# Dingyf717/target-allocation-ppo-transformer

Measured on AMD Instinct MI355X. Metric: env-steps/sec (whole node), full PPO rollout, 4096 envs x 16 UAV x 32 tgt per GPU, higher is better.
Workload: dtype f32 policy (f32 MFMA + fp32-accurate split products on the f16 MFMA) + f64 env

## Files before the change

target-allocation-ppo-transformer_amd/csrc/policy_block.hpp:

```cpp
#pragma once
#include "policy_encoder.hpp"

namespace uavhip {
namespace pol {

template <int head, int nout, int DQ = 4, int XT = (S - 1) * SPW>
__device__ void head_mlp(TID_F Smem& sm, const float* __restrict__ P, const APre<DQ>& pw, float* out) {
    const float* W0 = P + kOffs.o[head + 0];
    const float* b0 = P + kOffs.o[head + 1];
    const float* W2 = P + kOffs.o[head + 2];
    const float* b2 = P + kOffs.o[head + 3];
    const int wv = TIDX() >> 6;
    constexpr int kItems = SPW * nout;
    const int item = TIDX() >> 4, k4 = TIDX() & 15;
    const int p = item / nout, a = (item - p * nout) % nout;
    const f32x4 w2 = *reinterpret_cast<const f32x4*>(W2 + a * HID + 4 * k4);
    const float bb2 = b2[a];
    if (wv < HID / 16) linear1<1, true, DQ>(TID_C pw, W0, D, b0, 16 * wv, sm.h, LDH, XT, sm.z, LDZ, 16 * wv, 0);
    __syncthreads();
    if (item < kItems) {
        const f32x4 z = *reinterpret_cast<const f32x4*>(sm.z + p * LDZ + 4 * k4);
        float acc = (w2.x * z.x + w2.y * z.y) + (w2.z * z.z + w2.w * z.w);
        acc = add_xor2(add_xor1(acc));
        acc += __int_as_float(__builtin_amdgcn_mov_dpp(__float_as_int(acc), 0x141, 0xF, 0xF, true));
// ... 194 lines not shown
    static_assert(!AONLY || (ROWS && ENV && !TR && !VONLY), "actor only: the inference ring forward + env step");
    int blk = bx, role = VONLY ? 2 : AONLY ? 1 : 0;
    if constexpr (TR) {
        if (io.split) {
            role = blk < io.split ? 1 : 2;
            if (role == 2) blk -= io.split;
        }
    }
    const bool do_actor = role != 2, do_critic = role != 1;
    const int b0 = blk * SPW;
    [[maybe_unused]] bool critic_first = false;
    if constexpr (TR) critic_first = role == 0 && io.mix && ((blk >> 3) & 1);
    PTR(0);
    [[maybe_unused]] EmbPre ep_a, ep_c;
    [[maybe_unused]] KvPre<kActorTrunk, 0, TR> pkv_a;
    [[maybe_unused]] KvPre<kCriticTrunk, 0, TR> pkv_c;
    if constexpr (TR) {
        if (do_actor && !critic_first) {
            ep_a = embed_load<kActorTrunk>(TID_C P);
            pkv_a = kv_prefetch<kActorTrunk, 0, TR>(TID_C P);
        } else {
            ep_c = embed_load<kCriticTrunk>(TID_C P);
            pkv_c = kv_prefetch<kCriticTrunk, 0, TR>(TID_C P);
        }
    }
    gather_windows<TR, ROWS>(TID_C sm, states, B, io, b0, do_actor, P + kRangeOff);
    if constexpr (!TR) {
        const int pd = (int)TIDX() - (NTHR - kWave);
        if (!actions_in && pd >= 0 && pd < SPW) {
            const unsigned long long c = offset + (offset_dev ? *offset_dev : 0ull) + (unsigned long long)(b0 + pd);
            const u32x4 r = philox(u32x4{(uint32_t)c, (uint32_t)(c >> 32), 0x5eedu, 0x9e37u}, (uint32_t)seed,
                                   (uint32_t)(seed >> 32));
            sm.u01[pd] = u01f(r.x);
            if constexpr (AONLY) {
                if (greedy_stride > 0 && (b0 + pd) % greedy_stride == 0) sm.u01[pd] = -1.f;
            }
        }
    }
    __syncthreads();
    PTR(1);
    if (!ROWS || !do_actor) {
        const float xm = a0f_from_tmax(TID_C sm);
        if (TR && TIDX() == 0 && io.xmax) io.xmax[blk] = xm;
    }
    if (TR && blk == 0 && TIDX() < kRtN && io.rtab_out) io.rtab_out[TIDX()] = sm.rtab[TIDX()];
    const int wv = TIDX() >> 6;
    const float* headw_a = P + kOffs.o[kActorHead];
    const float* headw_c = P + kOffs.o[kCriticHead];
    [[maybe_unused]] const bool env_grp =
        (ENV & kEnvGrp) && env.N <= envgrp::L && env.M <= envgrp::L && b0 + 2 * wv + 1 < B;
    [[maybe_unused]] envgrp::GRegs gR;
    [[maybe_unused]] envgrp::GPending gq;
    if constexpr (ROWS) {
        if (do_actor) {
            RingPre<kActorTrunk> pw[3];
            RowPre<2> rp;
            rows_prologue<kActorTrunk>(TID_C sm, P, pw, rp, rio, b0, [&] { a0f_from_tmax(TID_C sm); });
            PTR(2);
            __syncthreads();
            encoder_layer_rows<kActorTrunk>(TID_C sm, P, pw, rp, rio, b0);
        }
    }
    constexpr int kHd = TR ? 2 : 4;
    APre<kHd> ph;
    [[maybe_unused]] auto actor = [&] {
        if constexpr (TR && !ROWS) {
            embed_apply<kActorTrunk, TR, kEmbH, split_kv<kActorTrunk, 0, TR>()>(TID_C sm, ep_a, io.e[0],
                                                                                           nullptr, b0);
            PTR(2);
            __syncthreads();
            auto hook = [&] {
                if (wv < 4) ph = prefetch<kHd>(TID_C headw_a, D, 16 * wv, 0);
                if (do_critic && !critic_first) {
                    ep_c = embed_load<kCriticTrunk>(TID_C P);
                    pkv_c = kv_prefetch<kCriticTrunk, 0, TR>(TID_C P);
                }
            };
            encoder_layer<kActorTrunk, 0, true, TR, decltype(hook)>(TID_C sm, P, pkv_a, io.L[0], b0, hook);
            __syncthreads();
            PTR(3);
            head_mlp<kActorHead, 2, kHd>(TID_C sm, P, ph, sm.logits);
            store_hidden(TID_C sm, io.z[0], b0);
        }
    };
    if constexpr (TR) {
        if (do_actor && !critic_first) actor();
    } else if (do_actor) {
        if constexpr (!ROWS) {
            APre<2> pkv = prefetch<2>(TID_C P + kOffs.o[layer_param(kActorTrunk, 0, INW)], D, kv_row(wv, 0), 0);
            embed<kActorTrunk, TR>(TID_C sm, P, io.e[0], nullptr, b0);
            PTR(2);
            __syncthreads();
            encoder_layer<kActorTrunk, 0, true, TR>(TID_C sm, P, pkv, io.L[0], b0);
        }
        if constexpr (AONLY && (ENV & kEnvGrp) && !kExpNoEnv) {
            if (env_grp) {
                const int le = tid_env() & 63;
                envgrp::gload_issue(gR, gq, env, b0 + 2 * (int)(tid_env() >> 6) + (le >> 5), le & 31);
            }
        }
        if (wv < 4) ph = prefetch<kHd>(TID_C headw_a, D, 16 * wv, 0);
        __syncthreads();
        PTR(3);
        head_mlp<kActorHead, 2, kHd>(TID_C sm, P, ph, sm.logits);
    }
    PTR(4);
    if (do_critic) {
// ... 166 lines not shown
```

target-allocation-ppo-transformer_amd/csrc/policy_encoder.hpp:

```cpp
#pragma once
#include "policy_core.hpp"

namespace uavhip {
namespace pol {

struct LnOut {
    float *x, *h, *rs;
    int b0, compact;
    bool nt = true;
};
__device__ __forceinline__ int trow(int tok, int b0) { return (b0 + (tok & (SPW - 1))) * S + tok / SPW; }
__device__ __forceinline__ int orow(int tok, int b0, bool compact) {
    return compact ? b0 + (tok & (SPW - 1)) : trow(tok, b0);
}

struct LnPar {
    f32x4 bb, ww, lb;
};
__device__ __forceinline__ f32x4 ln_bias(TID_F const float* __restrict__ bias) {
    return *reinterpret_cast<const f32x4*>(bias + 16 * (TIDX() >> 6) + 4 * (LANE() >> 4));
}
__device__ __forceinline__ LnPar ln_load(TID_F const f32x4 bb, const float* __restrict__ w, const float* __restrict__ b) {
    const int f0 = 16 * (TIDX() >> 6) + 4 * (LANE() >> 4);
    return LnPar{bb, *reinterpret_cast<const f32x4*>(w + f0), *reinterpret_cast<const f32x4*>(b + f0)};
// ... 130 lines not shown
        }
    }
}
__device__ __forceinline__ void attention_full_store(TID_F Smem& sm, int c, const f32x4 (&o)[3], float sc) {
    const int q4 = TIDX() & 3, task = TIDX() >> 2;
    const int hh = task & 3, p = (task >> 2) & 15, grp = task >> 6;
    const int d0 = hh * HD + 4 * q4, qs0 = grp ? 3 : 0, nq = grp ? 2 : 3;
#pragma unroll
    for (int qi = 0; qi < 3; ++qi) {
        if (qi < nq) {
            const int ti = (qs0 + qi) * SPW + p;
            hsplit_store(reinterpret_cast<_Float16*>(sm.ctx), psw(ti, 4 * c * HD + d0), o[qi] * sc);
        }
    }
}
template <int trunk, int layer>
__device__ void attention_full(TID_F Smem& sm, int c, const float* __restrict__ P = nullptr) {
    f32x4 o[3];
    attention_full_core(TID_C sm, c, o);
    attention_full_store(TID_C sm, c, o, att_sc<trunk, layer>(sm, (int)((TIDX() >> 4) & 15)).sc);
}

__device__ __forceinline__ void attention_task(TID_F Smem& sm, int task, int qs0, f32x4& o, int& ti, int& d0) {
    const int q4 = TIDX() & 3;
    const int hh = task & 3, rest = task >> 2, p = rest & 15, si = qs0 + (rest >> 4);
    ti = si * SPW + p;
    d0 = hh * HD + 4 * q4;
    const f32x4 q = *reinterpret_cast<const f32x4*>(sm.big + ti * LDB + d0) * kAttQ;
    float sc[S];
    float mx = -INFINITY;
#pragma unroll
    for (int j = 0; j < S; ++j) {
        const f32x4 k = *reinterpret_cast<const f32x4*>(sm.big + (j * SPW + p) * LDB + 64 + d0);
        float part = att_dot(q, k);
        part = add_xor2(add_xor1(part));
        sc[j] = sm.mask[p * S + j] ? -INFINITY : part;
        mx = j ? fmaxf(mx, sc[j]) : sc[j];
    }
    float den = 0.f;
#pragma unroll
    for (int j = 0; j < S; ++j) {
        sc[j] = __expf(sc[j] - mx);
        den = j ? den + sc[j] : sc[j];
    }
    const float inv = att_recip(den);
    f32x4 v[S];
#pragma unroll
    for (int j = 0; j < S; ++j) v[j] = *reinterpret_cast<const f32x4*>(sm.big + (j * SPW + p) * LDB + 128 + d0);
    o = f32x4{0.f, 0.f, 0.f, 0.f};
    att_mix(o, sc, inv, v);
}
__device__ __forceinline__ void attention_out(TID_F Smem& sm, int c, int ti, int d0, const f32x4 o, float sc) {
    hsplit_store(reinterpret_cast<_Float16*>(sm.ctx), psw(ti, 4 * c * HD + d0), o * sc);
}
template <int trunk, int layer>
__device__ void attention_chunk(TID_F Smem& sm, int c, int qs0, int nqs, const float* __restrict__ P = nullptr) {
    const int ntask = nqs * SPW * 4;
    for (int task = TIDX() >> 2; task < ntask; task += NTHR / 4) {
        f32x4 o;
        int ti, d0;
        attention_task(TID_C sm, task, qs0, o, ti, d0);
        attention_out(TID_C sm, c, ti, d0, o, att_sc<trunk, layer>(sm, ti & 15).sc);
    }
}

struct EmbPre {
    f32x4 a, bb, pp[S];
};
template <int trunk>
__device__ __forceinline__ EmbPre embed_load(TID_F const float* __restrict__ P) {
    const float* We = P + kOffs.o[trunk + EMB_W];
    const float* be = P + kOffs.o[trunk + EMB_B];
    const float* pos = P + kOffs.o[trunk + POS];
    const int l = LANE(), i16 = l & 15, g = l >> 4, wv = TIDX() >> 6;
    const int f = 16 * wv + i16;
    EmbPre r;
    r.a.x = 4 * g + 0 < IN ? We[f * IN + 4 * g + 0] : 0.f;
    r.a.y = 4 * g + 1 < IN ? We[f * IN + 4 * g + 1] : 0.f;
    r.a.z = 4 * g + 2 < IN ? We[f * IN + 4 * g + 2] : 0.f;
    r.a.w = 4 * g + 3 < IN ? We[f * IN + 4 * g + 3] : 0.f;
    r.bb = *reinterpret_cast<const f32x4*>(be + 16 * wv + 4 * g);
#pragma unroll
    for (int ct = 0; ct < S; ++ct) r.pp[ct] = *reinterpret_cast<const f32x4*>(pos + ct * D + 16 * wv + 4 * g);
    return r;
}
enum { kEmbH = 0, kEmbSplit = 1, kEmbRows = 2 };
template <int trunk, bool TR = false, int MODE = kEmbH, bool PL = false>
__device__ void embed_apply(TID_F Smem& sm, const EmbPre& ep, float* e_out = nullptr, float* h_out = nullptr, int b0 = 0) {
    const int l = LANE(), i16 = l & 15, g = l >> 4, wv = TIDX() >> 6;
    constexpr int NT = MODE == kEmbRows ? S - 1 : S;
    constexpr int CT0 = MODE == kEmbSplit && trunk == kActorTrunk ? S - 1 : 0;
    f32x4 acc[NT];
#pragma unroll
    for (int ct = CT0; ct < NT; ++ct) {
        const f32x4 b = *reinterpret_cast<const f32x4*>(sm.x + (ct * SPW + i16) * LDX + 4 * g);
        acc[ct] = f32x4{0.f, 0.f, 0.f, 0.f};
#pragma unroll
        for (int j = 0; j < 4; ++j) acc[ct] = __builtin_amdgcn_mfma_f32_16x16x4f32(ep.a[j], b[j], acc[ct], 0, 0, 0);
    }
#pragma unroll
    for (int ct = CT0; ct < NT; ++ct) {
        f32x4 e = acc[ct] + ep.bb;
        e.x = fmaxf(e.x, 0.f); e.y = fmaxf(e.y, 0.f); e.z = fmaxf(e.z, 0.f); e.w = fmaxf(e.w, 0.f);
        const int o = (ct * SPW + i16) * LDH + 16 * wv + 4 * g;
        constexpr bool ring_planes = split_slot(layer_param(trunk, 0, INW)) >= 0;
        const float esc = (ring_planes || PL) ? es_factor<trunk, -1>(sm, ct * SPW + i16) : 1.f;
        if ((MODE == kEmbRows || (MODE == kEmbSplit && ct == S - 1)) && ring_planes)
            hsplit_store(reinterpret_cast<_Float16*>(sm.ctx), psw((ct * SPW + i16), 16 * wv + 4 * g), e * esc);
        else if (MODE == kEmbRows || (MODE == kEmbSplit && ct == S - 1)) *reinterpret_cast<f32x4*>(sm.ctx + o) = e;
        if (MODE == kEmbRows) continue;
        const f32x4 v = e + ep.pp[ct];
        *reinterpret_cast<f32x4*>(sm.h + o) = v;
        if constexpr (PL) hsplit_store(reinterpret_cast<_Float16*>(sm.ctx), psw((ct * SPW + i16), 16 * wv + 4 * g), v * esc);
        if (TR) {
            const size_t r = (size_t)trow(ct * SPW + i16, b0);
            act_st(e_out + r * D + 16 * wv + 4 * g, e);
            if (h_out) act_st(h_out + r * D + 16 * wv + 4 * g, v);
        }
    }
}
template <int trunk, bool TR = false>
__device__ void embed(TID_F Smem& sm, const float* __restrict__ P, float* e_out = nullptr, float* h_out = nullptr,
                      int b0 = 0) {
    embed_apply<trunk, TR>(TID_C sm, embed_load<trunk>(TID_C P), e_out, h_out, b0);
}

__device__ __forceinline__ int kv_row(int wv, int c) { return (1 + (wv >> 2)) * D + 64 * c + 16 * (wv & 3); }

struct NoHook {
    __device__ void operator()() const {}
};
template <int trunk, int layer>
constexpr bool split_inproj() {
    return layer >= 1 && layer < 2 && split_slot(layer_param(trunk, layer, INW)) >= 0;
}
constexpr int kTailDepth = 2;
using TailPre = HPre<kTailDepth>;
template <int trunk, int layer, bool last, bool TR>
__device__ __forceinline__ TailPre tail_prefetch(TID_F const float* __restrict__ P) {
    const int wv = TIDX() >> 6;
    return hprefetch<kTailDepth>(TID_C P, split_slot(layer_param(trunk, layer, OUTW)), D, 16 * wv, 0);
}
template <int trunk, int layer, bool TR>
constexpr bool split_kv() {
    return split_inproj<trunk, layer>() || (TR && layer == 0);
}
template <int trunk, int layer, bool TR>
using KvPre = std::conditional_t<split_kv<trunk, layer, TR>(), HPre<2>, APre<2>>;
template <int trunk, int layer, bool TR>
__device__ __forceinline__ KvPre<trunk, layer, TR> kv_prefetch(TID_F const float* __restrict__ P) {
    const int wv = TIDX() >> 6;
    if constexpr (split_kv<trunk, layer, TR>())
        return hprefetch<2>(TID_C P, split_slot(layer_param(trunk, layer, INW)), D, kv_row(wv, 0), 0);
    else
        return prefetch<2>(TID_C P + kOffs.o[layer_param(trunk, layer, INW)], D, kv_row(wv, 0), 0);
}

__device__ __forceinline__ void store_qkv_chunk(TID_F const Smem& sm, float* __restrict__ qkv, int c, int qtok0, int b0) {
    for (int i = (int)TIDX() - NTHR / 2; i < TOK * 48; i += NTHR / 2) {
        if (i < 0) break;
// ... 80 lines not shown
    }
    PTR(tb + 8);
    __syncthreads();
    PTR(tb + 9);
    {
        const int grow = 4 * (LANE() >> 4);
        const f32x4 ba = *reinterpret_cast<const f32x4*>(b1 + 16 * wv + grow);
        const f32x4 bb = *reinterpret_cast<const f32x4*>(b1 + 128 + 16 * wv + grow);
        f32x4 hi[CT], lo[CT];
        zero(hi);
        zero(lo);
        HPre<DP> w1b;
        hgemm_tile<CT, DP, D / 32, LDP, kPlane, true>(TID_C hi, lo, w1a, P, s1, D, 16 * wv, 0, hp, t0, &w1b,
                                                      hfrag_ptr(TID_C P, s1, D, 128 + 16 * wv, 0));
        hstore_tile<CT, true>(TID_C hi, lo, ba, bp, 16 * wv, t0, s_ln1.inv, s_hid.sc);
        zero(hi);
        zero(lo);
        hgemm_tile<CT, DP>(TID_C hi, lo, w1b, P, s1, D, 128 + 16 * wv, 0, hp, t0);
        hstore_tile<CT, true>(TID_C hi, lo, bb, cp, 16 * wv, t0, s_ln1.inv, s_hid.sc);
    }
    const HPre<DP> w2a = hprefetch<DP>(TID_C P, s2, FF, 16 * wv, 0);
    PTR(tb + 10);
    __syncthreads();
    PTR(tb + 11);
    const HPre<DP> w2b = hprefetch<DP>(TID_C P, s2, FF, 16 * wv, 128);
    if constexpr (TR) {
        store_rows_planes(TID_C bp, io.u, FF, 0, D, t0, b0, last, t1, [&](int) { return s_hid.inv; }, !PSX);
        store_rows_planes(TID_C cp, io.u, FF, D, D, t0, b0, last, t1, [&](int) { return s_hid.inv; }, !PSX);
    }
    const LnPar lp2 = ln_load(TID_C ln_bias(TID_C b2), P + kOffs.o[layer_param(trunk, layer, N2W)],
                              P + kOffs.o[layer_param(trunk, layer, N2B)]);
    f32x4 hi[CT], lo[CT];
    zero(hi);
    zero(lo);
    hgemm_tile<CT, DP>(TID_C hi, lo, w2a, P, s2, FF, 16 * wv, 0, bp, t0);
    hgemm_tile<CT, DP>(TID_C hi, lo, w2b, P, s2, FF, 16 * wv, 128, cp, t0);
    PTR(tb + 12);
    f32x4 acc2[CT];
#pragma unroll
    for (int ct = 0; ct < CT; ++ct) acc2[ct] = (hi[ct] + lo[ct] * kLoScale) * s_hid.inv;
    pre_ln2();
    float ln2_sc = 1.f;
    if constexpr (next_planes) ln2_sc = op_sc<trunk, layer, kOpLn2>(sm).sc;
    residual_layernorm<CT, TR, next_planes, row4, kC0 ? 23 : -1, kC0 ? 39 : -1, kC0 ? 58 : -1>(
        TID_C sm, acc2, lp2, t0, LnOut{io.xhat2, PSX ? io.h2 : nullptr, io.rstd2, b0, last, !PSX}, nullptr, h1, ln2_sc);
    PTR(tb + 14);
}
template <int trunk, int layer, bool last, bool TR, class F = NoHook>
__device__ __forceinline__ void layer_tail_fwd(TID_F Smem& sm, const float* __restrict__ P, const TailPre& po,
                                               const TrainLayerIO& io, int b0, F pre_ln2 = F{}) {
    layer_tail<trunk, layer, last, TR, F>(TID_C sm, P, po, io, b0, pre_ln2);
}

template <int trunk, int layer, bool last, bool TR, class F = NoHook, bool TAIL = true>
__device__ __forceinline__ void encoder_layer_split(TID_F Smem& sm, const float* __restrict__ P, HPre<2> pkv,
                                                    const TrainLayerIO& io, int b0, F pre_ln2) {
    [[maybe_unused]] constexpr int tb = 8 + 16 * (trunk == 0 ? 0 : 1 + layer);
    PTR(tb);
    constexpr int si = split_slot(layer_param(trunk, layer, INW));
    constexpr int CTQ = last ? 1 : S, qtok0 = last ? (S - 1) * SPW : 0;
    constexpr bool in_ctx = layer == 0;
    static_assert(in_ctx || last, "a split in_proj after a full layer: a pruned layer");
    const float* bin = P + kOffs.o[layer_param(trunk, layer, INB)];
    const int l = LANE(), i16 = l & 15, g = l >> 4, wv = TIDX() >> 6;
    const _Float16* hp = reinterpret_cast<const _Float16*>(in_ctx ? sm.ctx : sm.h);
    TailPre po;
    [[maybe_unused]] f32x4 att0[last ? 1 : 3];
    [[maybe_unused]] int ti0 = 0, d00 = 0;
#pragma unroll
    for (int c = 0; c < 2; ++c) {
        HPre<2> pq;
        if (wv < 4) pq = hprefetch<2>(TID_C P, si, D, 64 * c + 16 * wv, 0);
        {
            const f32x4 bb = *reinterpret_cast<const f32x4*>(bin + kv_row(wv, c) + 4 * g);
            f32x4 hi[S], lo[S];
            zero(hi);
            zero(lo);
            hgemm_tile<S, 2>(TID_C hi, lo, pkv, P, si, D, kv_row(wv, c), 0, hp, 0);
            if constexpr (layer == 0) __asm__ volatile("" ::: "memory");
            const int col = (1 + (wv >> 2)) * 64 + 16 * (wv & 3) + 4 * g;
#pragma unroll
            for (int ct = 0; ct < S; ++ct)
                *reinterpret_cast<f32x4*>(sm.big + (16 * ct + i16) * LDB + col) =
                    (hi[ct] + lo[ct] * kLoScale) * in_inv<trunk, layer>(sm, 16 * ct + i16) + bb;
        }
        if (wv < 4) {
            const f32x4 bq = *reinterpret_cast<const f32x4*>(bin + 64 * c + 16 * wv + 4 * g);
            f32x4 hi[CTQ], lo[CTQ];
            zero(hi);
            zero(lo);
            hgemm_tile<CTQ, 2>(TID_C hi, lo, pq, P, si, D, 64 * c + 16 * wv, 0, hp, qtok0);
            if constexpr (layer == 0) __asm__ volatile("" ::: "memory");
#pragma unroll
            for (int ct = 0; ct < CTQ; ++ct)
                *reinterpret_cast<f32x4*>(sm.big + (qtok0 + 16 * ct + i16) * LDB + 16 * wv + 4 * g) =
                    (hi[ct] + lo[ct] * kLoScale) * in_inv<trunk, layer>(sm, qtok0 + 16 * ct + i16) + bq;
        }
        if (c == 0) pkv = hprefetch<2>(TID_C P, si, D, kv_row(wv, 1), 0);
        else if constexpr (TAIL) po = tail_prefetch<trunk, layer, last, TR>(TID_C P);
        PTR(tb + 1 + 3 * c);
        __syncthreads();
        PTR(tb + 2 + 3 * c);
        if constexpr (TR) store_qkv_chunk(TID_C sm, io.qkv, c, qtok0, b0);
        if constexpr (!in_ctx) {
            attention_chunk<trunk, layer>(TID_C sm, c, S - 1, 1, P);
        } else if constexpr (last) {
            f32x4 o;
            int ti = 0, d0 = 0;
            if (TIDX() < 4 * SPW * 4) attention_task(TID_C sm, TIDX() >> 2, S - 1, o, ti, d0);
            if (c == 0) {
                att0[0] = o;
                ti0 = ti;
                d00 = d0;
            } else if (TIDX() < 4 * SPW * 4) {
                const float asc = att_sc<trunk, layer>(sm, ti & 15).sc;
                attention_out(TID_C sm, 0, ti0, d00, att0[0], asc);
                attention_out(TID_C sm, 1, ti, d0, o, asc);
            }
        } else {
            if (c == 0) {
                attention_full_core(TID_C sm, 0, att0);
            } else {
                f32x4 o[3];
                attention_full_core(TID_C sm, 1, o);
                const float asc = att_sc<trunk, layer>(sm, (int)((TIDX() >> 4) & 15)).sc;
                attention_full_store(TID_C sm, 0, att0, asc);
                attention_full_store(TID_C sm, 1, o, asc);
            }
        }
        __syncthreads();
        PTR(tb + 3 + 3 * c);
    }
    if constexpr (TAIL) layer_tail_fwd<trunk, layer, last, TR, F>(TID_C sm, P, po, io, b0, pre_ln2);
}

template <int trunk, int layer, bool last, bool TR = false, class F = NoHook>
__device__ __forceinline__ void encoder_layer(TID_F Smem& sm, const float* __restrict__ P, KvPre<trunk, layer, TR> pkv,
                              const TrainLayerIO& io = TrainLayerIO{}, int b0 = 0, F pre_ln2 = F{}) {
    if constexpr (split_kv<trunk, layer, TR>()) {
        encoder_layer_split<trunk, layer, last, TR, F>(TID_C sm, P, pkv, io, b0, pre_ln2);
        return;
    } else {
    static_assert(!TR, "the training forward's in_proj GEMMs are split products");
    [[maybe_unused]] constexpr int tb = 8 + 16 * (trunk == 0 ? 0 : 1 + layer);
    PTR(tb);
    const float* Win = P + kOffs.o[layer_param(trunk, layer, INW)];
    const float* bin = P + kOffs.o[layer_param(trunk, layer, INB)];
    const int wv = TIDX() >> 6;
    constexpr int CTQ = last ? 1 : S;
    constexpr int DQ = depth<CTQ>();
    constexpr int qtok0 = last ? (S - 1) * SPW : 0;

    TailPre po;
#pragma unroll
    for (int c = 0; c < 2; ++c) {
        APre<DQ> pq;
        if (wv < 4) pq = prefetch<DQ>(TID_C Win, D, 64 * c + 16 * wv, 0);
        linear1<S, false, 2>(TID_C pkv, Win, D, bin, kv_row(wv, c), sm.h, LDH, 0, sm.big, LDB, (1 + (wv >> 2)) * 64 + 16 * (wv & 3), 0);
        if (wv < 4) linear1<CTQ, false, DQ>(TID_C pq, Win, D, bin, 64 * c + 16 * wv, sm.h, LDH, qtok0, sm.big, LDB, 16 * wv, qtok0);
        if (c == 0) pkv = prefetch<2>(TID_C Win, D, kv_row(wv, 1), 0);
        else po = tail_prefetch<trunk, layer, last, TR>(TID_C P);
        PTR(tb + 1 + 3 * c);
        __syncthreads();
        PTR(tb + 2 + 3 * c);
        if (last) attention_chunk<trunk, layer>(TID_C sm, c, S - 1, 1, P);
        else attention_full<trunk, layer>(TID_C sm, c, P);
        __syncthreads();
        PTR(tb + 3 + 3 * c);
    }
    layer_tail_fwd<trunk, layer, last, TR, F>(TID_C sm, P, po, io, b0, pre_ln2);
    }
}

constexpr int kPposFloats = 2 * S * 3 * D;
constexpr int kRowFloats = 5 * D;
struct RowIO {
    float* rp;
    int B, g;
};
constexpr int kPwD = 4;
template <int trunk> constexpr int row_parts() { return trunk == kActorTrunk ? 2 : 3; }
template <int NP>
struct RowPre {
    f32x4 v[2][2 * NP];
    float pp[2][2];
    f32x4 bias[3];
};

template <int trunk, int NP>
__device__ __forceinline__ void ppos_load(TID_F RowPre<NP>& r, const RowIO& rio) {
    const float* pp = rio.rp + (trunk == kActorTrunk ? 0 : S * 3 * D);
#pragma unroll
    for (int c = 0; c < 2; ++c)
#pragma unroll
        for (int u = 0; u < 2; ++u) {
            const int i = (TIDX() + NTHR * u) % (S * 192);
            const int s = i / 192, rr = i - 192 * s, part = rr >> 6, cc = rr & 63;
            r.pp[c][u] = pp[s * 3 * D + part * D + 64 * c + cc];
        }
}
template <int NP>
__device__ __forceinline__ void ppos_stage(TID_F Smem& sm, const RowPre<NP>& r, int c) {
    float* pl = reinterpret_cast<float*>(sm.red);
#pragma unroll
    for (int u = 0; u < 2; ++u) {
        const int i = TIDX() + NTHR * u;
        if (i < S * 192) pl[i] = r.pp[c][u];
    }
}
template <int NP>
__device__ __forceinline__ void ring_item(TID_F int u, int& part, int& tok) {
    const int t2 = (TIDX() >> 4) + 32 * u;
    part = t2 % NP;
    tok = t2 / NP;
}
template <int trunk, int NP>
__device__ __forceinline__ void ring_load(TID_F RowPre<NP>& r, const Smem& sm, const RowIO& rio, int b0, int c) {
    constexpr int ROFF = trunk == kActorTrunk ? 0 : 2 * D;
    const float* slots = rio.rp + kPposFloats;
    const int q = TIDX() & 15;
    int off[2 * NP];
#pragma unroll
    for (int u = 0; u < 2 * NP; ++u) {
        int part, tok;
        ring_item<NP>(TID_C u, part, tok);
        const int s = tok >> 4, p = tok & 15, b = b0 + p;
        const bool ok = b < rio.B && !sm.mask[p * S + s];
        const int slot = (rio.g + 1 + s) % 5;
        off[u] = ok ? (slot * rio.B + b) * kRowFloats + ROFF + part * D + 64 * c + 4 * q : -1;
    }
    __builtin_amdgcn_sched_barrier(0);
#pragma unroll
    for (int u = 0; u < 2 * NP; ++u) {
        const f32x4 v = *reinterpret_cast<const f32x4*>(slots + (off[u] >= 0 ? off[u] : 4 * q));
        r.v[c][u] = off[u] >= 0 ? v : f32x4{0.f, 0.f, 0.f, 0.f};
    }
}

template <int R, int D, class F>
__device__ __forceinline__ void gemm_rows(TID_F f32x4 (&acc)[R], const APre<D> (&pre)[R], const float* __restrict__ W,
                                          int ldw, const int (&row)[R], const float* X, int ldx, int xtok0,
                                          F&& issued) {
    const int l = LANE(), i16 = l & 15, g = l >> 4;
    const float* xp = X + (xtok0 + i16) * ldx + 4 * g;
    f32x4 a[KB][R], b[KB];
#pragma unroll
    for (int p = 0; p < D; ++p) {
#pragma unroll
        for (int r = 0; r < R; ++r) a[p][r] = pre[r].a[p];
        b[p] = *reinterpret_cast<const f32x4*>(xp + 16 * p);
    }
#pragma unroll
    for (int i = 0; i < KB; ++i) {
        if (i + D < KB) {
#pragma unroll
            for (int r = 0; r < R; ++r)
                a[i + D][r] = *reinterpret_cast<const f32x4*>(frag_ptr(TID_C W, ldw, row[r], 0) + 256 * (i + D));
            b[i + D] = *reinterpret_cast<const f32x4*>(xp + 16 * (i + D));
        }
        if (i == (D < KB ? KB - D - 1 : 0)) issued();
#pragma unroll
        for (int j = 0; j < 4; ++j)
#pragma unroll
            for (int r = 0; r < R; ++r) acc[r] = __builtin_amdgcn_mfma_f32_16x16x4f32(a[i][r][j], b[i][j], acc[r], 0, 0, 0);
        __builtin_amdgcn_sched_barrier(0);
    }
}

template <int R, int D_, class F>
__device__ __forceinline__ void hgemm_rows(TID_F f32x4 (&hi)[R], f32x4 (&lo)[R], const HPre<D_> (&pre)[R],
                                           const float* __restrict__ P, int soff, int K, const int (&row)[R],
                                           const _Float16* X, int xtok0, F&& issued) {
    constexpr int NKB = D / 32;
    const int l = LANE(), i16 = l & 15, g = l >> 4;
    const _Float16* xp = X + (xtok0 + i16) * LDP + 8 * (g ^ ((i16 >> 2) & 1));
    f16x8 a1[NKB][R], a2[NKB][R], b1[NKB], b2[NKB];
#pragma unroll
    for (int p = 0; p < D_; ++p)
#pragma unroll
        for (int r = 0; r < R; ++r) {
            a1[p][r] = pre[r].a1[p];
            a2[p][r] = pre[r].a2[p];
        }
    b1[0] = *reinterpret_cast<const f16x8*>(xp);
    b2[0] = *reinterpret_cast<const f16x8*>(xp + kPlane);
#pragma unroll
    for (int i = 0; i < NKB; ++i) {
        if (i + 1 < NKB) {
            b1[i + 1] = *reinterpret_cast<const f16x8*>(xp + 32 * (i + 1));
            b2[i + 1] = *reinterpret_cast<const f16x8*>(xp + 32 * (i + 1) + kPlane);
        }
        if (i + D_ < NKB) {
#pragma unroll
            for (int r = 0; r < R; ++r) {
                const f16x8* wp = hfrag_ptr(TID_C P, soff, K, row[r], 0) + 128 * (i + D_);
                a1[i + D_][r] = wp[0];
                a2[i + D_][r] = wp[64];
            }
        }
        if (i == (D_ < NKB ? NKB - D_ - 1 : 0)) issued();
#pragma unroll
        for (int r = 0; r < R; ++r) {
            hi[r] = __builtin_amdgcn_mfma_f32_16x16x32_f16(a1[i][r], b1[i], hi[r], 0, 0, 0);
            lo[r] = __builtin_amdgcn_mfma_f32_16x16x32_f16(a1[i][r], b2[i], lo[r], 0, 0, 0);
            lo[r] = __builtin_amdgcn_mfma_f32_16x16x32_f16(a2[i][r], b1[i], lo[r], 0, 0, 0);
        }
        __builtin_amdgcn_sched_barrier(0);
    }
}
template <int trunk>
constexpr bool split_ring() { return split_slot(layer_param(trunk, 0, INW)) >= 0; }
template <int trunk>
using RingPre = std::conditional_t<split_ring<trunk>(), HPre<2>, APre<kPwD>>;

template <int trunk, int NP>
__device__ __forceinline__ void encoder_layer_rows(TID_F Smem& sm, const float* __restrict__ P, const RingPre<trunk> (&pw)[3], RowPre<NP>& rp,
                                   const RowIO& rio, int b0) {
    constexpr bool last = trunk == kActorTrunk;
    constexpr int P0 = 3 - NP, ROFF = trunk == kActorTrunk ? 0 : 2 * D;
    [[maybe_unused]] constexpr int tb = 8 + 16 * (trunk == 0 ? 0 : 1);
    PTR(tb);
    const float* Win = P + kOffs.o[layer_param(trunk, 0, INW)];
    const int l = LANE(), i16 = l & 15, g = l >> 4, wv = TIDX() >> 6;
    const int rows[3] = {16 * wv, D + 16 * wv, 2 * D + 16 * wv};
    f32x4 acc[3] = {};
    auto ring_issue = [&] {
        ring_load<trunk>(TID_C rp, sm, rio, b0, 0);
        if (trunk == kActorTrunk) ring_load<trunk>(TID_C rp, sm, rio, b0, 1);
    };
    if constexpr (split_ring<trunk>()) {
        f32x4 lo[3] = {};
        const float inv = es_factor<trunk, 1>(sm, (S - 1) * SPW + i16);
        hgemm_rows<3, 2>(TID_C acc, lo, pw, P, split_slot(layer_param(trunk, 0, INW)), D, rows,
                         reinterpret_cast<const _Float16*>(sm.ctx), (S - 1) * SPW, ring_issue);
#pragma unroll
        for (int j = 0; j < 3; ++j) acc[j] = (acc[j] + lo[j] * kLoScale) * inv;
    } else {
        gemm_rows<3, kPwD>(TID_C acc, pw, Win, D, rows, sm.ctx, LDH, (S - 1) * SPW, ring_issue);
    }
#pragma unroll
    for (int j = 0; j < 3; ++j) acc[j] += rp.bias[j];
    if (b0 + i16 < rio.B) {
        float* dst = rio.rp + kPposFloats + ((size_t)(rio.g % 5) * rio.B + b0 + i16) * kRowFloats + ROFF + 16 * wv + 4 * g;
#pragma unroll
        for (int j = P0; j < 3; ++j) *reinterpret_cast<f32x4*>(dst + (j - P0) * D) = acc[j];
    }
    if (trunk != kActorTrunk) ring_load<trunk>(TID_C rp, sm, rio, b0, 1);
    PTR(tb + 13);
    const float* pl = reinterpret_cast<const float*>(sm.red);
    const int q = TIDX() & 15;
    TailPre po;
#pragma unroll
    for (int c = 0; c < 2; ++c) {
#pragma unroll
        for (int u = 0; u < 2 * NP; ++u) {
            int part, tok;
            ring_item<NP>(TID_C u, part, tok);
            const int bp = part + P0, s = tok >> 4;
            *reinterpret_cast<f32x4*>(sm.big + tok * LDB + bp * 64 + 4 * q) =
                rp.v[c][u] + *reinterpret_cast<const f32x4*>(pl + s * 192 + bp * 64 + 4 * q);
        }
        if ((wv >> 2) == c) {
#pragma unroll
            for (int j = 0; j < 3; ++j) {
                const int col = 64 * j + 16 * (wv & 3) + 4 * g;
                *reinterpret_cast<f32x4*>(sm.big + ((S - 1) * SPW + i16) * LDB + col) =
                    acc[j] + *reinterpret_cast<const f32x4*>(pl + (S - 1) * 192 + col);
            }
        }
        if (c == 1) po = tail_prefetch<trunk, 0, last, false>(TID_C P);
        PTR(tb + 1 + 3 * c);
        __syncthreads();
        PTR(tb + 2 + 3 * c);
        if (c == 0) ppos_stage(TID_C sm, rp, 1);
        if (last) attention_chunk<trunk, 0>(TID_C sm, c, S - 1, 1, P);
        else attention_full<trunk, 0>(TID_C sm, c, P);
        __syncthreads();
        PTR(tb + 3 + 3 * c);
    }
    layer_tail_fwd<trunk, 0, last, false>(TID_C sm, P, po, TrainLayerIO{}, b0);
}

template <int trunk, int NP, class H = NoHook>
__device__ __forceinline__ void rows_prologue(TID_F Smem& sm, const float* __restrict__ P, RingPre<trunk> (&pw)[3],
                                              RowPre<NP>& rp, const RowIO& rio, int b0, H hook = H{}) {
    const int wv = TIDX() >> 6;
    const EmbPre ep = embed_load<trunk>(TID_C P);
    ppos_load<trunk>(TID_C rp, rio);
    const float* Win = P + kOffs.o[layer_param(trunk, 0, INW)];
#pragma unroll
    for (int j = 0; j < 3; ++j) {
        if constexpr (split_ring<trunk>()) pw[j] = hprefetch<2>(TID_C P, split_slot(layer_param(trunk, 0, INW)), D, j * D + 16 * wv, 0);
        else pw[j] = prefetch<kPwD>(TID_C Win, D, j * D + 16 * wv, 0);
    }
    const float* bin = P + kOffs.o[layer_param(trunk, 0, INB)];
#pragma unroll
    for (int j = 0; j < 3; ++j) rp.bias[j] = *reinterpret_cast<const f32x4*>(bin + j * D + 16 * wv + 4 * (LANE() >> 4));
    hook();
    embed_apply<trunk, false, kEmbSplit>(TID_C sm, ep);
    ppos_stage(TID_C sm, rp, 0);
}

}
}
```

target-allocation-ppo-transformer_amd/csrc/rollout_steps.hip:

```cpp
#define UAVHIP_STEPS_TU 1
#define UAVHIP_TID_LAUNDER 1
#include "common.hpp"
#include "env_device.hpp"
#if defined(UAVHIP_POLICY_TRACE) && defined(UAVHIP_ENV_FINE)
namespace uavhip { namespace pol { __device__ unsigned long long g_strace[256 * 2 * 64]; } }
#define UAVHIP_STRACE_DEFINED 1
#define GTR(id)                                                                                  \
    do {                                                                                         \
        if ((tid_x() & 255) == 0 && blockIdx.x < 256)                                        \
            ::uavhip::pol::g_strace[(blockIdx.x * 2 + (tid_x() >> 8)) * 64 + (id)] = __builtin_amdgcn_s_memtime(); \
    } while (0)
#endif
#include "policy_steps.hpp"

namespace uavhip {
namespace pol {

#define UAVHIP_KARGS(Args)                                       \
    typedef const __attribute__((address_space(4))) Args* kargs; \
    kargs ka = (kargs)__builtin_amdgcn_kernarg_segment_ptr();    \
    int bx = blockIdx.x;                                         \
    unsigned tid = threadIdx.x;                                  \
    asm volatile("" : "+s"(ka), "+s"(bx), "+v"(tid));            \
    tid &= NTHR - 1;                                             \
// ... 105 lines not shown
        for (int i = tid; i < (a.n_max - t) * SPW; i += NTHR) {
            const int e = e0 + i % SPW;
            if (e < a.B) a.actions[(size_t)(t + i / SPW) * a.B + e] = -1;
        }
    }
}
int launch_decode_steps(const DecodeArgs& da, hipStream_t stream) {
    return launch_env_path<k_decode_steps<kEnvGrp>, k_decode_steps<kEnvWave>>(da, "k_decode_steps", stream);
}

template <int ENVP>
__global__ __launch_bounds__(NTHR) void k_rollout_actor_steps(const StepsArgs args) {
    __shared__ __attribute__((aligned(16))) Smem sm;
    if (threadIdx.x >= NTHR / 2) __builtin_amdgcn_s_setprio(1);
    if (threadIdx.x == 0) g_tid_zero = 0;
    load_rtab(TID_K sm, args.P);
    for (int t = 0; t < args.seq.n; ++t) {
        __syncthreads();
        UAVHIP_KARGS(StepsArgs);
        const size_t o = (size_t)t * a.B;
        const RowIO r{a.rio.rp, a.rio.B, a.rio.g + t};
        const EnvOut e{a.eo.auto_reset, a.eo.obs + t * a.seq.obs_stride, a.eo.rew + o, a.eo.done + o,
                       a.eo.info ? a.eo.info + o * UAVHIP_INFO_COUNT : nullptr};
        policy_block<false, true, ENVP, false, true, 1>(tid, sm, a.P, a.states + t * a.seq.obs_stride, a.B, nullptr,
                                                     a.seed, a.offset + t * a.seq.off_stride, a.offset_dev,
                                                     a.action_out + o, a.logp_out + o, nullptr, nullptr, nullptr,
                                                     TrainIO{}, r, a.env, e, bx, 0);
    }
}
int launch_rollout_actor_steps(const StepsArgs& sa, hipStream_t stream) {
    return launch_env_path<k_rollout_actor_steps<kEnvGrp>, k_rollout_actor_steps<kEnvWave>>(sa, "k_rollout_actor_steps",
                                                                                          stream);
}

constexpr int kStashVec = 2 * SPW * LDH / 4;
static_assert(LDP * 2 == LDH * 4, "a planes row and an fp32 row are the same bytes");
__device__ __forceinline__ void value_front(TID_F Smem& sm, const float* __restrict__ P, const float* __restrict__ states,
                                            int B, const RowIO& rio, int b0, f32x4* __restrict__ st) {
    PTR(0);
    gather_windows<false, true>(TID_C sm, states, B, TrainIO{}, b0, false, P + kRangeOff);
    __syncthreads();
    PTR(1);
    a0f_from_tmax(TID_C sm);
    {
        RingPre<kCriticTrunk> pw[3];
        RowPre<3> rp;
        rows_prologue<kCriticTrunk>(TID_C sm, P, pw, rp, rio, b0);
        PTR(2);
        __syncthreads();
        encoder_layer_rows<kCriticTrunk>(TID_C sm, P, pw, rp, rio, b0);
    }
    const KvPre<kCriticTrunk, 1, false> pkv = kv_prefetch<kCriticTrunk, 1, false>(TID_C P);
    __syncthreads();
    encoder_layer_split<kCriticTrunk, 1, true, false, NoHook, false>(TID_C sm, P, pkv, TrainLayerIO{}, b0, NoHook{});
    PTR(3);
    const f32x4* cx = reinterpret_cast<const f32x4*>(sm.ctx);
    for (int i = TIDX(); i < kStashVec; i += NTHR) {
        const int h = kStashVec / 2;
        st[i] = i < h ? cx[(S - 1) * SPW * LDH / 4 + i] : cx[i - h];
    }
    PTR(4);
}
template <int CT>
__device__ __forceinline__ void value_head_gemm(TID_F Smem& sm, const float* __restrict__ P, const APre<KB>& pw, int tok0) {
    const int row = 16 * ((TIDX() >> 6) & 3);
    linear1<CT, true, KB>(TID_C pw, P + kOffs.o[kCriticHead + 0], D, P + kOffs.o[kCriticHead + 1], row, sm.h, LDH, tok0,
                         sm.big, LDZ, row, tok0);
}
__global__ __launch_bounds__(NTHR) void k_value_steps(const ValueArgs args) {
    __shared__ __attribute__((aligned(16))) Smem sm;
    if (threadIdx.x >= NTHR / 2) __builtin_amdgcn_s_setprio(1);
    if (threadIdx.x == 0) g_tid_zero = 0;
    load_rtab(TID_K sm, args.P);
    const int nt = args.n + (args.last_values ? 1 : 0);
    for (int t0 = 0; t0 < nt; t0 += kVG) {
        for (int w = 0; w < kVG && t0 + w < nt; ++w) {
            __syncthreads();
            UAVHIP_KARGS(ValueArgs);
            const int t = t0 + w;
            const RowIO r{a.rio.rp, a.rio.B, a.rio.g + t};
            value_front(tid, sm, a.P, a.obs + t * a.obs_stride, a.B, r, bx * SPW,
                        reinterpret_cast<f32x4*>(a.stash) + ((size_t)bx * kVG + w) * kStashVec);
        }
        __syncthreads();
        UAVHIP_KARGS(ValueArgs);
        const int gw = min(kVG, nt - t0), b0 = bx * SPW;
        PTR(5);
        f32x4 res[kVG];
        {
            const f32x4* st = reinterpret_cast<const f32x4*>(a.stash) + (size_t)bx * kVG * kStashVec;
            constexpr int h = kStashVec / 2, kAll = kVG * h, kIt = (kAll + NTHR - 1) / NTHR;
            f32x4* cx = reinterpret_cast<f32x4*>(sm.ctx);
            f32x4 v[kIt];
#pragma unroll
            for (int u = 0; u < kIt; ++u) {
                const int i = min((int)tid + u * NTHR, kAll - 1), w = i / h;
                v[u] = st[w * kStashVec + (i - w * h)];
            }
            const int ro = h + (tid & 15) * (LDH / 4) + 4 * (tid >> 6) + ((tid >> 4) & 3);
#pragma unroll
            for (int w = 0; w < kVG; ++w) res[w] = st[w * kStashVec + ro];
            __builtin_amdgcn_sched_barrier(0);
#pragma unroll
            for (int u = 0; u < kIt; ++u) {
                const int i = tid + u * NTHR;
                if (i < kAll) cx[i] = i / h < gw ? v[u] : f32x4{0.f, 0.f, 0.f, 0.f};
            }
// ... 37 lines not shown
```

Before: 89.14 million.

## Add one-pass actor row layer and paired critic front attention

Adds an AONLY path for the actor's pruned row layer. It computes the new row's Q/K/V in one split GEMM from a single-row embedding in sm.big, gathers the cached K/V ring rows per lane, and runs the attention head in registers, avoiding the chunked attention loop and extra syncs. The critic's layer-1 front is replaced by encoder_front_pairs. It splits waves into K-scoring and V-holding halves, exchanges the softmax weights through shared memory and mixes them, which cuts GEMM passes and barriers. This adds register pressure and new shared-memory staging in sm.red and sm.big. It also removes the TAIL template flag.

```diff
diff --git a/target-allocation-ppo-transformer_amd/csrc/policy_block.hpp b/target-allocation-ppo-transformer_amd/csrc/policy_block.hpp
--- a/target-allocation-ppo-transformer_amd/csrc/policy_block.hpp
+++ b/target-allocation-ppo-transformer_amd/csrc/policy_block.hpp
@@ -270,7 +270,14 @@
     [[maybe_unused]] envgrp::GRegs gR;
     [[maybe_unused]] envgrp::GPending gq;
     if constexpr (ROWS) {
-        if (do_actor) {
+        if constexpr (AONLY) {
+            RingPre<kActorTrunk> pw[3];
+            RowPre1 rp;
+            rows_prologue_head(TID_C sm, P, pw, rp, rio, [&] { a0f_from_tmax(TID_C sm); });
+            PTR(2);
+            __syncthreads();
+            encoder_layer_rows<kActorTrunk, true>(TID_C sm, P, pw, rp, rio, b0);
+        } else if (do_actor) {
             RingPre<kActorTrunk> pw[3];
             RowPre<2> rp;
             rows_prologue<kActorTrunk>(TID_C sm, P, pw, rp, rio, b0, [&] { a0f_from_tmax(TID_C sm); });
diff --git a/target-allocation-ppo-transformer_amd/csrc/policy_encoder.hpp b/target-allocation-ppo-transformer_amd/csrc/policy_encoder.hpp
--- a/target-allocation-ppo-transformer_amd/csrc/policy_encoder.hpp
+++ b/target-allocation-ppo-transformer_amd/csrc/policy_encoder.hpp
@@ -206,6 +206,34 @@
 }
 __device__ __forceinline__ void attention_out(TID_F Smem& sm, int c, int ti, int d0, const f32x4 o, float sc) {
     hsplit_store(reinterpret_cast<_Float16*>(sm.ctx), psw(ti, 4 * c * HD + d0), o * sc);
+}
+__device__ __forceinline__ float attention_weights(TID_F const Smem& sm, const f32x4 q_, const f32x4 (&k)[S],
+                                                   float (&sc)[S]) {
+    const int p = LANE() & 15;
+    const f32x4 q = q_ * kAttQ;
+    float mx = -INFINITY;
+#pragma unroll
+    for (int j = 0; j < S; ++j) {
+        float part = att_dot(q, k[j]);
+        part = add_xor32(add_xor16(part));
+        sc[j] = sm.mask[p * S + j] ? -INFINITY : part;
+        mx = j ? fmaxf(mx, sc[j]) : sc[j];
+    }
+    float den = 0.f;
+#pragma unroll
+    for (int j = 0; j < S; ++j) {
+        sc[j] = __expf(sc[j] - mx);
+        den = j ? den + sc[j] : sc[j];
+    }
+    return att_recip(den);
+}
+__device__ __forceinline__ f32x4 attention_head(TID_F const Smem& sm, const f32x4 q_, const f32x4 (&k)[S],
+                                                const f32x4 (&v)[S]) {
+    float sc[S];
+    const float inv = attention_weights(TID_C sm, q_, k, sc);
+    f32x4 o = f32x4{0.f, 0.f, 0.f, 0.f};
+    att_mix(o, sc, inv, v);
+    return o;
 }
 template <int trunk, int layer>
 __device__ void attention_chunk(TID_F Smem& sm, int c, int qs0, int nqs, const float* __restrict__ P = nullptr) {
@@ -238,12 +266,14 @@
     for (int ct = 0; ct < S; ++ct) r.pp[ct] = *reinterpret_cast<const f32x4*>(pos + ct * D + 16 * wv + 4 * g);
     return r;
 }
-enum { kEmbH = 0, kEmbSplit = 1, kEmbRows = 2 };
+enum { kEmbH = 0, kEmbSplit = 1, kEmbRows = 2, kEmbOne = 3 };
 template <int trunk, bool TR = false, int MODE = kEmbH, bool PL = false>
 __device__ void embed_apply(TID_F Smem& sm, const EmbPre& ep, float* e_out = nullptr, float* h_out = nullptr, int b0 = 0) {
     const int l = LANE(), i16 = l & 15, g = l >> 4, wv = TIDX() >> 6;
     constexpr int NT = MODE == kEmbRows ? S - 1 : S;
-    constexpr int CT0 = MODE == kEmbSplit && trunk == kActorTrunk ? S - 1 : 0;
+    constexpr int CT0 = (MODE == kEmbSplit || MODE == kEmbOne) && trunk == kActorTrunk ? S - 1 : 0;
+    static_assert(MODE != kEmbOne || (trunk == kActorTrunk && split_slot(layer_param(trunk, 0, INW)) >= 0),
+                  "the actor's one-pass step: a split new-row GEMM");
     f32x4 acc[NT];
 #pragma unroll
     for (int ct = CT0; ct < NT; ++ct) {
@@ -259,7 +289,9 @@
         const int o = (ct * SPW + i16) * LDH + 16 * wv + 4 * g;
         constexpr bool ring_planes = split_slot(layer_param(trunk, 0, INW)) >= 0;
         const float esc = (ring_planes || PL) ? es_factor<trunk, -1>(sm, ct * SPW + i16) : 1.f;
-        if ((MODE == kEmbRows || (MODE == kEmbSplit && ct == S - 1)) && ring_planes)
+        if (MODE == kEmbOne && ct == S - 1)
+            hsplit_store(reinterpret_cast<_Float16*>(sm.big), psw(i16, 16 * wv + 4 * g), e * esc);
+        else if ((MODE == kEmbRows || (MODE == kEmbSplit && ct == S - 1)) && ring_planes)
             hsplit_store(reinterpret_cast<_Float16*>(sm.ctx), psw((ct * SPW + i16), 16 * wv + 4 * g), e * esc);
         else if (MODE == kEmbRows || (MODE == kEmbSplit && ct == S - 1)) *reinterpret_cast<f32x4*>(sm.ctx + o) = e;
         if (MODE == kEmbRows) continue;
@@ -446,7 +478,7 @@
     layer_tail<trunk, layer, last, TR, F>(TID_C sm, P, po, io, b0, pre_ln2);
 }
 
-template <int trunk, int layer, bool last, bool TR, class F = NoHook, bool TAIL = true>
+template <int trunk, int layer, bool last, bool TR, class F = NoHook>
 __device__ __forceinline__ void encoder_layer_split(TID_F Smem& sm, const float* __restrict__ P, HPre<2> pkv,
                                                     const TrainLayerIO& io, int b0, F pre_ln2) {
     [[maybe_unused]] constexpr int tb = 8 + 16 * (trunk == 0 ? 0 : 1 + layer);
@@ -491,7 +523,7 @@
                     (hi[ct] + lo[ct] * kLoScale) * in_inv<trunk, layer>(sm, qtok0 + 16 * ct + i16) + bq;
         }
         if (c == 0) pkv = hprefetch<2>(TID_C P, si, D, kv_row(wv, 1), 0);
-        else if constexpr (TAIL) po = tail_prefetch<trunk, layer, last, TR>(TID_C P);
+        else po = tail_prefetch<trunk, layer, last, TR>(TID_C P);
         PTR(tb + 1 + 3 * c);
         __syncthreads();
         PTR(tb + 2 + 3 * c);
@@ -525,7 +557,68 @@
         __syncthreads();
         PTR(tb + 3 + 3 * c);
     }
-    if constexpr (TAIL) layer_tail_fwd<trunk, layer, last, TR, F>(TID_C sm, P, po, io, b0, pre_ln2);
+    layer_tail_fwd<trunk, layer, last, TR, F>(TID_C sm, P, po, io, b0, pre_ln2);
+}
+
+constexpr int kAttW = 8;
+template <int trunk, int layer>
+__device__ __forceinline__ void encoder_front_pairs(TID_F Smem& sm, const float* __restrict__ P, HPre<2> pkv) {
+    static_assert(split_inproj<trunk, layer>(), "the input's planes in sm.h: a pruned layer after a full one");
+    constexpr int si = split_slot(layer_param(trunk, layer, INW));
+    constexpr int qtok0 = (S - 1) * SPW;
+    const float* bin = P + kOffs.o[layer_param(trunk, layer, INB)];
+    const int l = LANE(), i16 = l & 15, g = l >> 4, wv = TIDX() >> 6, h = wv & 3;
+    const _Float16* hp = reinterpret_cast<const _Float16*>(sm.h);
+    f32x4 v[S];
+#pragma unroll
+    for (int c = 0; c < 2; ++c) {
+        const bool kw = (wv < 4) == (c == 0);
+        const int row = (kw ? D : 2 * D) + 64 * c + 16 * h;
+        HPre<2> pq;
+        if (kw) pq = hprefetch<2>(TID_C P, si, D, 64 * c + 16 * h, 0);
+        f32x4 t[S];
+        {
+            const f32x4 bb = *reinterpret_cast<const f32x4*>(bin + row + 4 * g);
+            f32x4 hi[S], lo[S];
+            zero(hi);
+            zero(lo);
+            hgemm_tile<S, 2>(TID_C hi, lo, pkv, P, si, D, row, 0, hp, 0);
+#pragma unroll
+            for (int ct = 0; ct < S; ++ct)
+                t[ct] = (hi[ct] + lo[ct] * kLoScale) * in_inv<trunk, layer>(sm, 16 * ct + i16) + bb;
+        }
+        if (kw) {
+            const f32x4 bq = *reinterpret_cast<const f32x4*>(bin + 64 * c + 16 * h + 4 * g);
+            f32x4 hi[1], lo[1];
+            zero(hi);
+            zero(lo);
+            hgemm_tile<1, 2>(TID_C hi, lo, pq, P, si, D, 64 * c + 16 * h, 0, hp, qtok0);
+            const f32x4 q = (hi[0] + lo[0] * kLoScale) * in_inv<trunk, layer>(sm, qtok0 + i16) + bq;
+            float e[S];
+            const float inv = attention_weights(TID_C sm, q, t, e);
+            if (g == 0) {
+                float* w = sm.big + ((c * 4 + h) * SPW + i16) * kAttW;
+                *reinterpret_cast<f32x4*>(w) = f32x4{e[0], e[1], e[2], e[3]};
+                *reinterpret_cast<f32x2_t*>(w + 4) = f32x2_t{e[4], inv};
+            }
+        } else {
+#pragma unroll
+            for (int ct = 0; ct < S; ++ct) v[ct] = t[ct];
+        }
+        if (c == 0) pkv = hprefetch<2>(TID_C P, si, D, (wv < 4 ? 2 * D : D) + 64 + 16 * h, 0);
+    }
+    __syncthreads();
+    {
+        const int c = wv < 4 ? 1 : 0;
+        const float* w = sm.big + ((c * 4 + h) * SPW + i16) * kAttW;
+        const f32x4 e4 = *reinterpret_cast<const f32x4*>(w);
+        const f32x2_t e1 = *reinterpret_cast<const f32x2_t*>(w + 4);
+        const float e[S] = {e4.x, e4.y, e4.z, e4.w, e1.x};
+        f32x4 o = f32x4{0.f, 0.f, 0.f, 0.f};
+        att_mix(o, e, e1.y, v);
+        attention_out(TID_C sm, c, qtok0 + i16, 16 * h + 4 * g, o, att_sc<trunk, layer>(sm, i16).sc);
+    }
+    __syncthreads();
 }
 
 template <int trunk, int layer, bool last, bool TR = false, class F = NoHook>
@@ -631,6 +724,49 @@
     }
 }
 
+struct RowPre1 {
+    f32x4 v[S - 1][2];
+    int ok;
+    f32x4 pt;
+    f32x4 pq;
+    f32x4 bias[3];
+};
+constexpr int kPpos1Vec = S * 2 * D / 4;
+static_assert(kPpos1Vec * 4 * sizeof(float) == sizeof(Smem::red) && kPpos1Vec <= NTHR, "the K | V table in sm.red");
+__device__ __forceinline__ void ppos_load_head(TID_F RowPre1& r, const RowIO& rio) {
+    const float* pp = rio.rp;
+    const int i = TIDX() % kPpos1Vec;
+    r.pt = *reinterpret_cast<const f32x4*>(pp + (i >> 6) * 3 * D + D + 4 * (i & 63));
+    r.pq = *reinterpret_cast<const f32x4*>(pp + (S - 1) * 3 * D + 16 * (TIDX() >> 6) + 4 * (LANE() >> 4));
+}
+__device__ __forceinline__ void ppos_stage_head(TID_F Smem& sm, const RowPre1& r) {
+    if (TIDX() < kPpos1Vec) reinterpret_cast<f32x4*>(sm.red)[TIDX()] = r.pt;
+}
+__device__ __forceinline__ void ring_load_head(TID_F RowPre1& r, const Smem& sm, const RowIO& rio, int b0) {
+    const float* slots = rio.rp + kPposFloats;
+    const int p = LANE() & 15, b = b0 + p;
+    const int col = 16 * (int)(TIDX() >> 6) + 4 * (LANE() >> 4);
+    int off[S - 1], m[S - 1];
+#pragma unroll
+    for (int s = 0; s < S - 1; ++s) m[s] = sm.mask[p * S + s];
+    r.ok = 0;
+#pragma unroll
+    for (int s = 0; s < S - 1; ++s) {
+        const bool ok = (b < rio.B) & (m[s] == 0);
+        const int slot = (rio.g + 1 + s) % 5;
+        off[s] = ok ? (slot * rio.B + b) * kRowFloats + col : col;
+        r.ok |= (int)ok << s;
+    }
+    __builtin_amdgcn_sched_barrier(0);
+#pragma unroll
+    for (int s = 0; s < S - 1; ++s)
+#pragma unroll
+        for (int part = 0; part < 2; ++part) r.v[s][part] = *reinterpret_cast<const f32x4*>(slots + off[s] + part * D);
+}
+__device__ __forceinline__ f32x4 ring_value(const RowPre1& r, int s, int part) {
+    return (r.ok >> s) & 1 ? r.v[s][part] : f32x4{0.f, 0.f, 0.f, 0.f};
+}
+
 template <int R, int D, class F>
 __device__ __forceinline__ void gemm_rows(TID_F f32x4 (&acc)[R], const APre<D> (&pre)[R], const float* __restrict__ W,
                                           int ldw, const int (&row)[R], const float* X, int ldx, int xtok0,
@@ -707,10 +843,13 @@
 template <int trunk>
 using RingPre = std::conditional_t<split_ring<trunk>(), HPre<2>, APre<kPwD>>;
 
-template <int trunk, int NP>
-__device__ __forceinline__ void encoder_layer_rows(TID_F Smem& sm, const float* __restrict__ P, const RingPre<trunk> (&pw)[3], RowPre<NP>& rp,
+template <int trunk, bool ONEPASS = false, class RP>
+__device__ __forceinline__ void encoder_layer_rows(TID_F Smem& sm, const float* __restrict__ P, const RingPre<trunk> (&pw)[3], RP& rp,
                                    const RowIO& rio, int b0) {
     constexpr bool last = trunk == kActorTrunk;
+    constexpr int NP = row_parts<trunk>();
+    static_assert(std::is_same_v<RP, std::conditional_t<ONEPASS, RowPre1, RowPre<NP>>>, "the variant's ring operands");
+    static_assert(!ONEPASS || (last && split_ring<trunk>()), "one pass: the actor's pruned layer, split new-row GEMM");
     constexpr int P0 = 3 - NP, ROFF = trunk == kActorTrunk ? 0 : 2 * D;
     [[maybe_unused]] constexpr int tb = 8 + 16 * (trunk == 0 ? 0 : 1);
     PTR(tb);
@@ -719,14 +858,19 @@
     const int rows[3] = {16 * wv, D + 16 * wv, 2 * D + 16 * wv};
     f32x4 acc[3] = {};
     auto ring_issue = [&] {
-        ring_load<trunk>(TID_C rp, sm, rio, b0, 0);
-        if (trunk == kActorTrunk) ring_load<trunk>(TID_C rp, sm, rio, b0, 1);
+        if constexpr (ONEPASS) {
+            ring_load_head(TID_C rp, sm, rio, b0);
+        } else {
+            ring_load<trunk>(TID_C rp, sm, rio, b0, 0);
+            if (trunk == kActorTrunk) ring_load<trunk>(TID_C rp, sm, rio, b0, 1);
+        }
     };
     if constexpr (split_ring<trunk>()) {
         f32x4 lo[3] = {};
         const float inv = es_factor<trunk, 1>(sm, (S - 1) * SPW + i16);
         hgemm_rows<3, 2>(TID_C acc, lo, pw, P, split_slot(layer_param(trunk, 0, INW)), D, rows,
-                         reinterpret_cast<const _Float16*>(sm.ctx), (S - 1) * SPW, ring_issue);
+                         reinterpret_cast<const _Float16*>(ONEPASS ? sm.big : sm.ctx), ONEPASS ? 0 : (S - 1) * SPW,
+                         ring_issue);
 #pragma unroll
         for (int j = 0; j < 3; ++j) acc[j] = (acc[j] + lo[j] * kLoScale) * inv;
     } else {
@@ -734,11 +878,41 @@
     }
 #pragma unroll
     for (int j = 0; j < 3; ++j) acc[j] += rp.bias[j];
+    if constexpr (!ONEPASS) {
     if (b0 + i16 < rio.B) {
         float* dst = rio.rp + kPposFloats + ((size_t)(rio.g % 5) * rio.B + b0 + i16) * kRowFloats + ROFF + 16 * wv + 4 * g;
 #pragma unroll
         for (int j = P0; j < 3; ++j) *reinterpret_cast<f32x4*>(dst + (j - P0) * D) = acc[j];
     }
+    }
+    if constexpr (ONEPASS) {
+        PTR(tb + 13);
+        const TailPre po = tail_prefetch<trunk, 0, last, false>(TID_C P);
+        const float* pl = reinterpret_cast<const float*>(sm.red) + 16 * wv + 4 * g;
+        f32x4 k[S], v[S];
+#pragma unroll
+        for (int s = 0; s < S - 1; ++s) {
+            k[s] = ring_value(rp, s, 0);
+            v[s] = ring_value(rp, s, 1);
+        }
+        k[S - 1] = acc[1];
+        v[S - 1] = acc[2];
+#pragma unroll
+        for (int s = 0; s < S; ++s) {
+            k[s] += *reinterpret_cast<const f32x4*>(pl + s * 2 * D);
+            v[s] += *reinterpret_cast<const f32x4*>(pl + s * 2 * D + D);
+        }
+        const f32x4 o = attention_head(TID_C sm, acc[0] + rp.pq, k, v);
+        attention_out(TID_C sm, 0, (S - 1) * SPW + i16, 16 * wv + 4 * g, o, att_sc<trunk, 0>(sm, i16).sc);
+        if (b0 + i16 < rio.B) {
+            float* dst = rio.rp + kPposFloats + ((size_t)(rio.g % 5) * rio.B + b0 + i16) * kRowFloats + 16 * wv + 4 * g;
+            *reinterpret_cast<f32x4*>(dst) = acc[1];
+            *reinterpret_cast<f32x4*>(dst + D) = acc[2];
+        }
+        __syncthreads();
+        PTR(tb + 3);
+        layer_tail_fwd<trunk, 0, last, false>(TID_C sm, P, po, TrainLayerIO{}, b0);
+    } else {
     if (trunk != kActorTrunk) ring_load<trunk>(TID_C rp, sm, rio, b0, 1);
     PTR(tb + 13);
     const float* pl = reinterpret_cast<const float*>(sm.red);
@@ -773,6 +947,7 @@
         PTR(tb + 3 + 3 * c);
     }
     layer_tail_fwd<trunk, 0, last, false>(TID_C sm, P, po, TrainLayerIO{}, b0);
+    }
 }
 
 template <int trunk, int NP, class H = NoHook>
@@ -794,6 +969,23 @@
     embed_apply<trunk, false, kEmbSplit>(TID_C sm, ep);
     ppos_stage(TID_C sm, rp, 0);
 }
-
-}
-}
+template <class H = NoHook>
+__device__ __forceinline__ void rows_prologue_head(TID_F Smem& sm, const float* __restrict__ P,
+                                                   RingPre<kActorTrunk> (&pw)[3], RowPre1& rp, const RowIO& rio,
+                                                   H hook = H{}) {
+    constexpr int trunk = kActorTrunk;
+    const int wv = TIDX() >> 6;
+    const EmbPre ep = embed_load<trunk>(TID_C P);
+    ppos_load_head(TID_C rp, rio);
+#pragma unroll
+    for (int j = 0; j < 3; ++j) pw[j] = hprefetch<2>(TID_C P, split_slot(layer_param(trunk, 0, INW)), D, j * D + 16 * wv, 0);
+    const float* bin = P + kOffs.o[layer_param(trunk, 0, INB)];
+#pragma unroll
+    for (int j = 0; j < 3; ++j) rp.bias[j] = *reinterpret_cast<const f32x4*>(bin + j * D + 16 * wv + 4 * (LANE() >> 4));
+    hook();
+    embed_apply<trunk, false, kEmbOne>(TID_C sm, ep);
+    ppos_stage_head(TID_C sm, rp);
+}
+
+}
+}
diff --git a/target-allocation-ppo-transformer_amd/csrc/rollout_steps.hip b/target-allocation-ppo-transformer_amd/csrc/rollout_steps.hip
--- a/target-allocation-ppo-transformer_amd/csrc/rollout_steps.hip
+++ b/target-allocation-ppo-transformer_amd/csrc/rollout_steps.hip
@@ -181,7 +181,7 @@
     }
     const KvPre<kCriticTrunk, 1, false> pkv = kv_prefetch<kCriticTrunk, 1, false>(TID_C P);
     __syncthreads();
-    encoder_layer_split<kCriticTrunk, 1, true, false, NoHook, false>(TID_C sm, P, pkv, TrainLayerIO{}, b0, NoHook{});
+    encoder_front_pairs<kCriticTrunk, 1>(TID_C sm, P, pkv);
     PTR(3);
     const f32x4* cx = reinterpret_cast<const f32x4*>(sm.ctx);
     for (int i = TIDX(); i < kStashVec; i += NTHR) {
```

Measured after the change: 90.92 million (median of 6 runs). 2.0% higher.
